# a-to-the-5/Simple-MapReduce-Search-Engine-Information-Retrieval-

Measured on AMD Instinct MI355X. Metric: index build GB/s of text (top-10 queries/sec in 'query'), higher is better.
Workload: dtype u8 text / int32 postings / f64 weights

## Files before the change

### simple-mapreduce-search-engine-information-retrieval-_amd/csrc/sme_api.hip

```cpp
#include <hip/hip_runtime.h>
#include <string.h>

#include <sstream>
#include <string>
#include <vector>

#include <algorithm>
#include <system_error>
#include <thread>

#include "sme_feedback.hpp"
#include "sme_internal.hpp"

namespace {
thread_local std::string g_err;

int fail(int code, const std::string &msg) {
  g_err = msg;
  return code;
}

template <typename F>
int guard(F &&f) {
  try {
// ... 245 lines not shown
      range(0, 2);
      cx->opt_query_kernel = v;
    } else if (n == "heavy_div") {
      range(0, int64_t(1) << 40);
      cx->opt_heavy_div = v;
    } else if (n == "seed_tiles") {
      range(0, 8);
      cx->opt_seed_tiles = v;
    } else if (n == "query_order") {
      range(0, 1);
      cx->opt_query_order = v;
    } else if (n == "agg_two_pass") {
      range(0, 1);
      cx->opt_agg_two_pass = v;
    } else if (n == "agg_grid") {
      range(0, int64_t(1) << 30);
      cx->opt_agg_grid = v;
    } else if (n == "tok_grid") {
      range(1, int64_t(1) << 30);
      cx->opt_tok_grid = v;
    } else if (n == "cand_cap") {
      range(1, 2048);
      cx->opt_cand_cap = v;
    } else if (n == "win_sample") {
      range(0, 1);
      cx->opt_win_sample = v;
    } else if (n == "win_stage_min") {
      range(0, int64_t(1) << 20);
      cx->opt_win_stage_min = v;
    } else if (n == "kgram_rank") {
      range(0, 1);
      cx->opt_kgram_rank = v;
    } else if (n == "win_slice") {
      range(0, int64_t(1) << 30);
      cx->opt_win_slice = v;
    } else if (n == "seed_m") {
      range(0, 4096);
      cx->opt_seed_m = v;
    } else if (n == "query_table_budget") {
      range(0, int64_t(1) << 50);
      cx->opt_query_budget = v;
    } else if (n == "corpus_keep_bytes") {
      range(0, int64_t(1) << 50);
      cx->opt_corpus_keep = v;
    } else if (n == "raw_load_pct") {
      range(10, 90);
      cx->opt_raw_load_pct = v;
    } else if (n == "docid_terms") {
      range(0, 1);
      cx->opt_docid_terms = v;
    } else if (n == "sort_digit_bits") {
      if (v != 0) range(6, 11);
      cx->opt_sort_bits = v;
    } else if (n == "docid_split") {
      range(0, 2);
      cx->opt_docid_split = v;
    } else if (n == "wild_scan") {
      range(0, 1);
      cx->opt_wild_scan = v;
    } else if (n == "wild_chunk") {
      range(64, 4096);
      if (v % 64) throw sme::Error(SME_EINVAL, "option " + n + " must be a multiple of 64");
      cx->opt_wild_chunk = v;
    } else if (n == "fuzzy_scan") {
      range(0, 1);
      cx->opt_fuzzy_scan = v;
    } else if (n == "bool_chunk") {
      range(64, 4096);
      if (v % 64) throw sme::Error(SME_EINVAL, "option " + n + " must be a multiple of 64");
      cx->opt_bool_chunk = v;
    } else if (n == "bool_driver") {
      range(0, 1);
      cx->opt_bool_driver = v;
    } else if (n == "positions") {
      range(0, 1);
      cx->opt_positions = v;
    } else if (n == "struct_narrow") {
      range(0, 1);
      cx->opt_struct_narrow = v;
    } else if (n == "fb_slots") {
      if (!sme::feedback::legal_slots(v))
        throw sme::Error(SME_EINVAL, "option " + n + " must be a power of two in [" +
                                         std::to_string(sme::feedback::kMinSlots) + ", " +
                                         std::to_string(sme::feedback::kMaxSlots) + "]");
      cx->opt_fb_slots = v;
    } else {
      throw sme::Error(SME_EINVAL, "unknown option " + n);
    }
  });
}

static void ctx_release(sme_ctx *cx) {
  (void)hipSetDevice(cx->device);
  (void)hipDeviceSynchronize();
  if (cx->own_stream) (void)hipStreamDestroy(cx->own_stream);
  if (cx->aux_stream) (void)hipStreamDestroy(cx->aux_stream);
  if (cx->ev_fork) (void)hipEventDestroy(cx->ev_fork);
  if (cx->ev_join) (void)hipEventDestroy(cx->ev_join);
  for (hipEvent_t e : cx->prof_events) (void)hipEventDestroy(e);
  for (auto &b : cx->h_stage)
    if (b) (void)hipHostFree(b);
  delete cx;
}

void sme_destroy(sme_ctx *cx) {
  if (!cx) return;
// ... 952 lines not shown
```

### simple-mapreduce-search-engine-information-retrieval-_amd/csrc/sme_build.hip

```cpp
#include <hip/hip_runtime.h>
#include <limits.h>
#include <math.h>
#include <stdio.h>
#include <stdlib.h>
#include <string.h>

#include <algorithm>
#include <memory>
#include <chrono>

#include "sme_internal.hpp"
#include "sme_text.hpp"
#include "sme_trec.hpp"

namespace sme {


template <typename B>
__device__ bool doc_tag_valid(const B &t, int64_t p, const char *tag, int tl) {
  int chain = 0;
  int64_t x = p;
  for (;;) {
    int64_t q = -1;
    for (int j = 1; j < tl; j++) {
// ... 1952 lines not shown
    raw_nout[s] = 1;
  }
}

__global__ void k_code_to_merged(int32_t *raw_term, uint64_t rcap, int32_t *multi, int64_t nmulti,
                                 const int64_t *wrank, const int64_t *drank) {
  const uint64_t gs = (uint64_t)gridDim.x * blockDim.x;
  for (uint64_t s = blockIdx.x * (uint64_t)blockDim.x + threadIdx.x; s < rcap + (uint64_t)nmulti; s += gs) {
    int32_t *p = s < rcap ? raw_term + s : multi + (s - rcap);
    const int32_t v = *p;
    if (v >= 0) *p = (int32_t)((v & kDocCode) ? drank[v & ~kDocCode] : wrank[v]);
  }
}
__global__ void k_dsplit_flags(const int32_t *dk_rec, int64_t nR, uint8_t *flag) {
  for (int64_t i = blockIdx.x * (int64_t)blockDim.x + threadIdx.x; i < nR; i += (int64_t)gridDim.x * blockDim.x)
    flag[i] = dk_rec[i] >= 0;
}
__global__ void k_dsplit_gather(const int32_t *idx, const unsigned long long *nd, const int32_t *dk_rec,
                                const uint32_t *dv_rec, uint32_t *dk, uint32_t *dv, unsigned long long *desc) {
  const int64_t n = (int64_t)*nd;
  for (int64_t q = blockIdx.x * (int64_t)blockDim.x + threadIdx.x; q < n; q += (int64_t)gridDim.x * blockDim.x) {
    dk[q] = (uint32_t)dk_rec[idx[q]];
    dv[q] = dv_rec[idx[q]];
    if (q > 0 && dk_rec[idx[q - 1]] > dk_rec[idx[q]]) atomicAdd(desc, 1ull);
  }
}
__global__ void k_word_shift(const int64_t *wrank, int64_t Vw, const uint32_t *dk, int64_t Nd, uint2 *ws) {
  for (int64_t i = blockIdx.x * (int64_t)blockDim.x + threadIdx.x; i < Vw; i += (int64_t)gridDim.x * blockDim.x) {
    const uint32_t below = (uint32_t)(wrank[i] - i);
    int64_t lo = 0, hi = Nd;
    while (lo < hi) {
      const int64_t m = (lo + hi) >> 1;
      if (dk[m] < below) lo = m + 1;
      else hi = m;
    }
    ws[i] = make_uint2((uint32_t)lo, (uint32_t)wrank[i]);
  }
}
__device__ __forceinline__ int64_t words_below(int64_t j, const int64_t *drank, const int64_t *wrank, int64_t Vw,
                                               const uint2 *ws, const int64_t *off, int64_t Pw) {
  const int64_t x = drank[j] - j;
  return x < Vw ? off[wrank[x]] - (int64_t)ws[x].x : Pw;
}
__global__ void k_docid_place(const uint32_t *dk, const uint32_t *dv, int64_t Nd, const int64_t *drank,
                              const int64_t *wrank, int64_t Vw, const uint2 *ws, const int64_t *off, int64_t Pw,
                              int64_t dmin, uint32_t F, int32_t *docno, int32_t *tf, uint32_t *key, const double *lut,
                              double idf, double *w) {
  for (int64_t q = blockIdx.x * (int64_t)blockDim.x + threadIdx.x; q < Nd; q += (int64_t)gridDim.x * blockDim.x) {
    const int64_t j = dk[q];
    const int64_t p = q + words_below(j, drank, wrank, Vw, ws, off, Pw);
    const uint32_t v = dv[q];
    docno[p] = (int32_t)((int64_t)(v / F) + dmin);
    tf[p] = (int32_t)(v % F);
    key[p] = (uint32_t)drank[j];
    if (w) w[p] = __dmul_rn(lut[v % F], idf);
  }
}
__global__ void k_docid_off(const uint32_t *dk, int64_t Nd, int64_t Vd, const int64_t *drank, const int64_t *wrank,
                            int64_t Vw, const uint2 *ws, int64_t Pw, int64_t *off) {
  for (int64_t j = blockIdx.x * (int64_t)blockDim.x + threadIdx.x; j < Vd; j += (int64_t)gridDim.x * blockDim.x) {
    int64_t lo = 0, hi = Nd;
    while (lo < hi) {
      const int64_t m = (lo + hi) >> 1;
      if ((int64_t)dk[m] < j) lo = m + 1;
      else hi = m;
    }
    off[drank[j]] = lo + words_below(j, drank, wrank, Vw, ws, off, Pw);
  }
}

constexpr int kAggNT = 256;
constexpr int kAggCap = 4096;
constexpr int kAggLimit = 3072;

__device__ __forceinline__ uint32_t hash32(uint32_t x) {
  x ^= x >> 16;
  x *= 0x7feb352dU;
  x ^= x >> 15;
  x *= 0x846ca68bU;
  x ^= x >> 16;
  return x;
}

__device__ __forceinline__ bool agg_insert(int32_t *keys, int32_t *cnt, uint32_t cap_mask, int32_t term,
                                           int32_t *distinct, int32_t limit) {
  uint32_t h = hash32((uint32_t)term) & cap_mask;
  for (uint32_t probe = 0; probe <= cap_mask; probe++) {
    int32_t old = atomicCAS(&keys[h], -1, term);
    if (old == -1) {
      int32_t d = atomicAdd(distinct, 1);
      atomicAdd(&cnt[h], 1);
      return d < limit;
    }
    if (old == term) {
      atomicAdd(&cnt[h], 1);
      return true;
    }
    h = (h + 1) & cap_mask;
  }
  return false;
}

struct AggIn {
  const uint64_t *rs;
  const uint32_t *tokstream;
  const int32_t *ntok;
  const int32_t *raw_term;
// ... 1685 lines not shown
  int64_t Pm = P;
  int32_t max_tf = 1;
  bool packed = false;
  int64_t dmin = 0;
  uint32_t F = 0;
  if (ai.v32 != nullptr || ai.rec_val != nullptr) {
    max_tf = std::max<int32_t>(1, h_mtf);
    packed = true;
    dmin = ai.dmin;
    F = ai.F;
  } else if (P > 0 && !dup_docno && K == 1) {
    SME_HIP(hipMemsetAsync(mtf, 0, sizeof(unsigned int), st));
    const int h_init[2] = {INT_MAX, INT_MIN};
    SME_HIP(hipMemcpyAsync(dmn, h_init, sizeof h_init, hipMemcpyHostToDevice, st));
    hipLaunchKernelGGL(k_pair_stats, dim3(grid_for(P, 256, 2048)), dim3(256), 0, st, p_val, P, mtf);
    hipLaunchKernelGGL(k_docno_range, dim3(grid_for(nR, 256, 1024)), dim3(256), 0, st, docno, nR, dmn, dmx);
    unsigned int h_m = d2h(mtf, st);
    int h_r[2];
    SME_HIP(hipMemcpyAsync(h_r, dmn, sizeof h_r, hipMemcpyDeviceToHost, st));
    SME_HIP(hipStreamSynchronize(st));
    const uint64_t Fq = (uint64_t)h_m + 1, D = (uint64_t)((int64_t)h_r[1] - (int64_t)h_r[0] + 1);
    max_tf = std::max<int32_t>(1, (int32_t)h_m);
    packed = D * Fq < (1ull << 32) && tbits + bits_for((uint64_t)max_tf) <= 32;
    dmin = h_r[0];
    F = (uint32_t)Fq;
  }
  int32_t *docno_d = nullptr, *tf_d = nullptr;
  int64_t *off = nullptr;
  std::vector<double> early_lut;
  bool weights_fused = false;
  if (packed) {
    const int sort_bits = cx->opt_sort_bits > 0 ? (int)cx->opt_sort_bits : (Pw > (int64_t(1) << 30) ? 8 : 11);
    uint32_t *v32 = ai.v32;
    if (ai.rec_val != nullptr) {
      if (term_sort_passes(tbits, sort_bits) >= 3) v32 = W[W_PVAL].as<uint32_t>(P + 1);
    } else if (v32 == nullptr) {
      v32 = reinterpret_cast<uint32_t *>(W[W_T1].as<uint64_t>(P + 1));
      hipLaunchKernelGGL(k_pack_pairs, dim3(grid_for(P)), dim3(256), 0, st, p_val, P, dmin, F, v32);
    }
    uint32_t *v32s = W[W_T2].as<uint32_t>(P + 1);
    docno_d = ix->d_docno_d.as<int32_t>(P + 1);
    tf_d = ix->d_tf_d.as<int32_t>(P + 1);
    uint32_t *rscr = W[W_RADIX].as<uint32_t>(term_sort_scratch(P) / sizeof(uint32_t) + 1);
    double *wf = nullptr;
    if (ix->idf_mode == SME_IDF_REFERENCE && P > 0) {
      early_lut.assign((size_t)max_tf + 1, 0.0);
      for (int i = 1; i <= max_tf; i++) early_lut[(size_t)i] = 1.0 + log((double)i);
      SME_HIP(hipMemcpyAsync(ix->d_lut.as<double>(max_tf + 1), early_lut.data(), early_lut.size() * sizeof(double),
                             hipMemcpyHostToDevice, st));
      wf = ix->d_w.as<double>(P + 1);
      weights_fused = true;
    }
    const double idf_r = log10((double)(std::max<int64_t>(nR, 0) / 1));
    key_s = term_sort(p_term, v32, key_s, v32s, sort_nrec, sort_reg, sort_xoff, Pw, tbits, dmin, F, docno_d, tf_d, rscr,
                      st, wf ? (const double *)ix->d_lut.p : nullptr, idf_r, wf, sort_bits, xw, P, ai.rec_val,
                      ai.tf_shift);
    off = ix->d_off.as<int64_t>(Vi + 1);
    SME_HIP(hipMemsetAsync(off, 0, (Vi + 1) * sizeof(int64_t), st));
    if (!split) {
      hipLaunchKernelGGL(k_term_offsets<false>, dim3(grid_for(P)), dim3(256), 0, st, key_s, P, off, Vi);
    } else {
      hipLaunchKernelGGL(k_term_offsets<true>, dim3(grid_for(P)), dim3(256), 0, st, key_s, P, off, Vi);
      hipLaunchKernelGGL(k_docid_off, dim3(grid_for(Vd)), dim3(256), 0, st, dk, Nd, Vd, (const int64_t *)drank,
                         (const int64_t *)wrank_all, Vw, xw, Pw, off);
      if (Nd > 0)
        hipLaunchKernelGGL(k_docid_place, dim3(grid_for(Nd)), dim3(256), 0, st, dk, dv, Nd, (const int64_t *)drank,
                           (const int64_t *)wrank_all, Vw, xw, off, Pw, dmin, F, docno_d, tf_d, key_s,
                           wf ? (const double *)ix->d_lut.p : nullptr, idf_r, wf);
    }
    SME_CHECK_LAUNCH();
  } else {
    uint64_t *val_s = W[W_T1].as<uint64_t>(P + 1);
    if (P > 0)
      sort_pairs_v64<uint32_t>(p_term, key_s, p_val, val_s, P, tbits, cx->ws[120], cx->ws[121], cx->ws[122], st);
    if (dup_docno && P > 0) {
      uint64_t *ck = W[W_PVAL].as<uint64_t>(P), *ck2 = W[W_T2].as<uint64_t>(P);
      int32_t *tfv = reinterpret_cast<int32_t *>(W[W_PTERM].as<uint32_t>(P)), *tf2 = W[W_T3].as<int32_t>(P);
      hipLaunchKernelGGL(k_dup_keys, dim3(grid_for(P)), dim3(256), 0, st, key_s, val_s, P, ck, tfv);
      int64_t *nout = reinterpret_cast<int64_t *>(cnt + 10);
      reduce_by_key_sum(ck, tfv, P, ck2, tf2, nout, cx->ws[120], cx->ws[121], cx->ws[23], st);
      Pm = d2h(nout, st);
      hipLaunchKernelGGL(k_dup_unpack, dim3(grid_for(Pm)), dim3(256), 0, st, ck2, tf2, Pm, key_s, val_s);
    }
    off = ix->d_off.as<int64_t>(Vi + 1);
    SME_HIP(hipMemsetAsync(off, 0, (Vi + 1) * sizeof(int64_t), st));
    if (Pm > 0) hipLaunchKernelGGL(k_term_offsets<false>, dim3(grid_for(Pm)), dim3(256), 0, st, key_s, Pm, off, Vi);
    docno_d = ix->d_docno_d.as<int32_t>(Pm + 1);
    tf_d = ix->d_tf_d.as<int32_t>(Pm + 1);
    if (Pm > 0) hipLaunchKernelGGL(k_unpack_vals, dim3(grid_for(Pm)), dim3(256), 0, st, val_s, Pm, docno_d, tf_d);
    SME_CHECK_LAUNCH();
    if (Pm > 0) {
      int32_t *mx = reinterpret_cast<int32_t *>(cnt + 11);
      reduce_max<int32_t>(tf_d, Pm, mx, st);
      max_tf = std::max(1, d2h(mx, st));
    }
  }
  ix->P = Pm;
  const int64_t PP = Pm;
  prof.mark("sort_term");

  ix->max_tf = max_tf;
  {
    std::vector<double> lut(max_tf + 1, 0.0);
    for (int i = 1; i <= max_tf; i++) lut[i] = 1.0 + log((double)i);
    double *d_lut = ix->d_lut.as<double>(max_tf + 1);
    SME_HIP(hipMemcpyAsync(d_lut, lut.data(), lut.size() * sizeof(double), hipMemcpyHostToDevice, st));
    const int64_t Nn = std::max<int64_t>(nR, 0);
    ix->idf_N = Nn;
    double idf_ref = idf_value(Nn, 1);
    int64_t sdf = (int64_t)std::sqrt((double)std::max<int64_t>(Nn, 1)) + 1;
    std::vector<double> by_df(sdf + 1), by_q(Nn / std::max<int64_t>(sdf, 1) + 2);
    for (int64_t d = 1; d <= sdf; d++) by_df[d] = idf_value(Nn, d);
    for (size_t q = 0; q < by_q.size(); q++) by_q[q] = idf_value((int64_t)q, 1);
    double *d_bydf = W[W_U16].as<double>(by_df.size() + by_q.size());
    double *d_byq = d_bydf + by_df.size();
    SME_HIP(hipMemcpyAsync(d_bydf, by_df.data(), by_df.size() * sizeof(double), hipMemcpyHostToDevice, st));
    SME_HIP(hipMemcpyAsync(d_byq, by_q.data(), by_q.size() * sizeof(double), hipMemcpyHostToDevice, st));
    double *idf = ix->d_idf.as<double>(Vi + 1);
    if (Vi > 0)
      hipLaunchKernelGGL(k_term_idf, dim3(grid_for(Vi)), dim3(256), 0, st, off, Vi, idf_ref, Nn, nullptr, d_bydf, sdf,
                         d_byq, ix->idf_mode, idf);
// ... 123 lines not shown
```

### simple-mapreduce-search-engine-information-retrieval-_amd/csrc/sme_internal.hpp

```cpp
#pragma once
#include <hip/hip_runtime.h>
#include <math.h>
#include <stdint.h>

#include <memory>
#include <string>
#include <vector>

#include "sme_common.hpp"
#include "sme_result.hpp"

struct sme_ctx {
  sme::BufPool pool;
  sme_config cfg{};
  int device = 0;
  hipStream_t own_stream = nullptr;
  hipStream_t aux_stream = nullptr;
  hipEvent_t ev_fork = nullptr, ev_join = nullptr;
  std::vector<hipEvent_t> prof_events;
  sme::DevBuf map_chars, map_off;
  int64_t map_n = 0;
  bool has_map = false;
  sme::DevBuf map_slots;
  uint64_t map_mask = 0;
  bool map_hash_ok = false;
  sme::DevBuf ws[128];
  sme::DevBuf cub_tmp;
  sme::DevBuf q_gates;
  uint64_t vocab_long_cap = 0, vocab_ovf_cap = 0, raw_cap_hint = 0, lt_cap_hint = 0;
  std::string profile_json;
  std::vector<std::pair<std::string, float>> last_profile;
  std::vector<uint8_t> mapping_out;
  std::vector<int32_t> h_wlist;
  float last_query_ms = -1.0f;
  float last_query_prep_ms = -1.0f;
  float last_query_index_ms = -1.0f;
  bool last_query_tiled = false;
  const char *last_query_name = "k_query";
  float last_query_seed_ms = 0.0f, last_query_final_ms = 0.0f, last_query_total_ms = 0.0f;
  int64_t last_query_overflow = 0;
  int64_t last_query_fallback = 0;
  int64_t last_query_stages = 0;
  int64_t last_query_slices = 0;
  bool last_query_split = false;
  int64_t opt_query_kernel = 0;
  int64_t opt_heavy_div = 128;
  int64_t opt_seed_tiles = 4;
  int64_t opt_query_order = 1;
  int64_t opt_agg_two_pass = 0;
  int64_t opt_agg_grid = 0;
  int64_t opt_tok_grid = 5120;
  int64_t opt_raw_load_pct = 40;
  int64_t opt_docid_terms = 1;
  int64_t opt_sort_bits = 0;
  int64_t opt_docid_split = 1;
  int64_t opt_cand_cap = 1024;
  int64_t opt_seed_m = 64;
  int64_t opt_kgram_rank = 0;
  int64_t opt_win_slice = 0;
  int64_t opt_win_sample = 1;
  int64_t opt_win_stage_min = 0;
  int64_t opt_query_budget = 0;
  int64_t opt_wild_scan = 0;
  int64_t opt_wild_chunk = 1024;
  int64_t opt_fuzzy_scan = 0;
  int64_t opt_bool_chunk = 1024;
  int64_t opt_bool_driver = 0;
  int64_t opt_positions = 0;
  int64_t opt_struct_narrow = 1;
  int64_t opt_fb_slots = 4096;
  int64_t opt_corpus_keep = int64_t(16) << 30;
  void *h_stage[2] = {nullptr, nullptr};
  size_t h_stage_cap = 0;
  sme::DevBuf h_corpus_dev;
  int live_indexes = 0;
  bool destroyed = false;
};

struct sme_index {
  sme_ctx *ctx = nullptr;
  int K = 1, R = 1, idf_mode = 0;
  int job = 0;
  int64_t cg_ngrams = 0, cg_pairs = 0;
  int64_t N = 0, V = 0, P = 0;
  int64_t Vt = 0;
  int32_t max_tf = 0;
  int64_t dmin = 0, dmax = -1;
  sme::DevBuf d_term_off;
  sme::DevBuf d_term_chars;
  sme::DevBuf d_off;
  sme::DevBuf d_docno_d;
  sme::DevBuf d_tf_d;
  sme::DevBuf d_w;
  sme::DevBuf d_idf;
  sme::DevBuf d_gram;
  sme::DevBuf d_lut;
  sme::DevBuf d_docno_o;
  sme::DevBuf d_tf_o;
  sme::DevBuf d_rec_docno;
  sme::DevBuf d_rec_first;
  bool records_only = false;
  bool from_records = false;
  sme::DevBuf d_ser;
  std::vector<int64_t> part_start;
  bool ser_ready = false;
  float ser_ms = 0.0f;
  std::vector<std::unique_ptr<uint8_t[]>> h_parts;
// ... 64 lines not shown
  std::vector<hipEvent_t> *pool;
  std::vector<std::pair<std::string, hipEvent_t>> ev;
  Prof(hipStream_t s, std::vector<hipEvent_t> *p) : st(s), pool(p) { mark("start"); }
  ~Prof() {
    for (auto &e : ev) pool->push_back(e.second);
  }
  void mark(const char *name) {
    hipEvent_t e;
    if (!pool->empty()) {
      e = pool->back();
      pool->pop_back();
    } else {
      SME_HIP(hipEventCreate(&e));
    }
    ev.emplace_back(name, e);
    last_stage() = name;
    SME_HIP(hipEventRecord(e, st));
  }
  std::vector<std::pair<std::string, float>> finish() {
    SME_HIP(hipEventSynchronize(ev.back().second));
    std::vector<std::pair<std::string, float>> out;
    for (size_t i = 1; i < ev.size(); i++) {
      float ms = 0;
      SME_HIP(hipEventElapsedTime(&ms, ev[i - 1].second, ev[i].second));
      out.emplace_back(ev[i].first, ms);
    }
    float tot = 0;
    SME_HIP(hipEventElapsedTime(&tot, ev.front().second, ev.back().second));
    out.emplace_back("total", tot);
    for (auto &p : ev) pool->push_back(p.second);
    ev.clear();
    return out;
  }
};

struct RecordSpans {
  uint64_t *rs, *re;
  int64_t nR;
  uint64_t *C;
  int64_t nC;
  int lt_attempts;
};
void build_docid_hash(sme_ctx *cx, bool distinct, hipStream_t st);
RecordSpans find_records(sme_ctx *cx, const uint8_t *d_text, uint64_t n, hipStream_t st, Prof *prof);
void split_points(sme_ctx *cx, const uint8_t *d_text, uint64_t n, int world, uint64_t *h_cuts, hipStream_t st);
void number_documents(sme_ctx *cx, const uint8_t *d_text, uint64_t n, hipStream_t st, std::vector<uint8_t> &out);
sme_index *build_index(sme_ctx *cx, const uint8_t *d_text, uint64_t n, hipStream_t st, int job = 0);
void chargram_stage(sme_ctx *cx, sme_index *ix, const int32_t *tstream, int64_t M, int64_t V, const int64_t *term_off,
                    const uint16_t *term_chars, hipStream_t st, Prof *prof);
uint32_t *term_sort(uint32_t *k0, uint32_t *v0, uint32_t *k1, uint32_t *v1, int64_t nrec, const int64_t *reg,
                    const int64_t *xoff, int64_t P, int bits, int64_t dmin, uint32_t F, int32_t *docno, int32_t *tf,
                    uint32_t *counts, hipStream_t st, const double *lut = nullptr, double idf = 0.0,
                    double *w = nullptr, int maxbits = 11, const uint2 *xw = nullptr, int64_t Pout = 0,
                    const uint32_t *rec_val = nullptr, int tf_shift = 0);
int term_sort_passes(int bits, int maxbits);
size_t term_sort_scratch(int64_t P);
template <typename K>
uint32_t *kv_sort(K *k0, uint32_t *v0, K *k1, uint32_t *v1, int64_t n, int bits, uint32_t *scratch, hipStream_t st,
                  bool keys_out = false);
size_t kv_sort_scratch(int64_t n);
template <typename T>
void excl_scan(const T *in, T *out, int64_t n, DevBuf &scratch, hipStream_t st);
void select_flagged(const uint8_t *flag, int64_t n, int32_t *out, int32_t *d_count, DevBuf &s1, DevBuf &s2,
                    hipStream_t st);
template <typename K>
void sort_pairs(K *keys_in, K *keys_out, uint32_t *vals_in, uint32_t *vals_out, int64_t n, int bits, DevBuf &radix,
                hipStream_t st);
template <typename K>
void sort_pairs_v64(K *keys_in, K *keys_out, const uint64_t *vals_in, uint64_t *vals_out, int64_t n, int bits,
                    DevBuf &ia, DevBuf &ib, DevBuf &radix, hipStream_t st);
template <typename T>
void reduce_max(const T *in, int64_t n, T *d_max, hipStream_t st);
void reduce_by_key_sum(const uint64_t *keys, const int32_t *vals, int64_t n, uint64_t *ukeys, int32_t *sums,
                       int64_t *d_runs, DevBuf &flags, DevBuf &pos, DevBuf &scan, hipStream_t st);
constexpr int kTfSortMaxTf = 1023;
void tf_sort_segments(const int64_t *off, int64_t V, int64_t P, const int32_t *docno_d, const int32_t *tf_d,
                      int max_tf, int32_t *docno_o, int32_t *tf_o, DevBuf &lists, DevBuf &tiles, DevBuf &tcnt, DevBuf &scan,
                      unsigned long long *nseg, hipStream_t st, hipStream_t aux_stream, hipEvent_t ev_fork,
                      hipEvent_t ev_join);
void serialize_index(sme_index *ix, hipStream_t st);
void pack_pieces(sme_index *ix, int world, uint8_t *d_out, uint64_t *sizes, hipStream_t st);
sme_index *merge_pieces(sme_ctx *cx, const uint8_t *d_blobs, const uint64_t *sizes, int np, hipStream_t st);
void reweight_index(sme_index *ix, int64_t N, const int64_t *d_gdf, hipStream_t st,
                    const uint32_t *d_term_of = nullptr);
sme_index *load_records(sme_ctx *cx, const uint8_t *d_records, const uint64_t *part_offsets, int np, hipStream_t st);
void prepare_queries(sme_index *ix, hipStream_t st);
void query_topk(sme_index *ix, const int32_t *d_terms, const int64_t *d_qoff, int nq, int k,
                int32_t *d_out_docno, double *d_out_score, uint32_t *d_out_tie, hipStream_t st, int tie_bits = 0);
void query_topk_java7(sme_index *ix, const int32_t *d_terms, const int64_t *d_qoff, int nq, int k,
                      int32_t *d_out_docno, double *d_out_score, uint32_t *d_out_tie, hipStream_t st);
void tokenize_string(sme_ctx *cx, const uint8_t *h_utf8, size_t n, std::vector<std::vector<uint16_t>> &out,
                     hipStream_t st);
void term_fingerprints(sme_index *ix, uint64_t *d_out, hipStream_t st);
void dfx_pack(sme_ctx *cx, const uint64_t *fp, const int64_t *df, int64_t n, int world, uint64_t *sfp, int64_t *sdf,
              int64_t *pos, int64_t *h_counts, hipStream_t st);
void dfx_sum(sme_ctx *cx, const uint64_t *fp, const int64_t *df, int64_t n, int64_t *out, int64_t *h_distinct,
             hipStream_t st);
void dfx_unpack(const int64_t *ret, const int64_t *pos, int64_t n, int64_t *out, hipStream_t st);
void merge_rows(const double *s, const int32_t *d, const uint32_t *t, int64_t rows, int m, int k, int32_t *od,
                double *os, uint32_t *ot, hipStream_t st);
int64_t count_shared_keys(sme_ctx *cx, const uint64_t *rows, int64_t n, hipStream_t st);
void lookup_terms(sme_index *ix, const std::vector<std::vector<uint16_t>> &terms, int32_t *ids,
                  hipStream_t st);
void prepare_wildcards(sme_index *ix, hipStream_t st);
void expand_wildcards(sme_index *ix, const uint8_t *patterns, const int64_t *offs, int n, hipStream_t st);
void suggest_terms(sme_index *ix, const uint8_t *words, const int64_t *offs, int n, int max_dist, int m,
                   hipStream_t st);
// ... 26 lines not shown
```

### simple-mapreduce-search-engine-information-retrieval-_amd/csrc/sme_sort.hip

```cpp
#include <hip/hip_runtime.h>

#include "sme_internal.hpp"

namespace sme {
namespace {

#ifndef SME_RSNT
#define SME_RSNT 512
#endif
constexpr int kRsNT = SME_RSNT;
constexpr int kRsWaves = kRsNT / 64;
constexpr int kRsIPL = 16;
constexpr int kRsTile = kRsNT * kRsIPL;
constexpr int kRsWaveItems = 64 * kRsIPL;
constexpr int kRsMaxBits = 11;
constexpr int kRsMaxBins = 1 << kRsMaxBits;
constexpr int kRsBPT = kRsMaxBins / kRsNT;
constexpr int kRsGroups = 1024;
constexpr int kRsScanSums = 1024;

struct RsGroups {
  int64_t tpg;
  int G;
};
static RsGroups rs_groups(int64_t ntiles) {
  const int64_t tpg = std::max<int64_t>(4, (ntiles + kRsGroups - 1) / kRsGroups);
  const int64_t g = (ntiles + tpg - 1) / tpg;
  return RsGroups{tpg, (int)((g + 15) / 16 * 16)};
}

struct Gather {
  const int64_t *reg, *xoff, *crec;
  int64_t nrec;
  const uint32_t *rval;
  int tf_shift;
};
__device__ __forceinline__ void gather_start(const Gather &g, int64_t x, int64_t &rec, int64_t &nx, int64_t &dl) {
  rec = g.crec[x >> 10];
  nx = g.xoff[rec + 1];
  dl = g.reg[rec] - g.xoff[rec];
}
__device__ __forceinline__ int64_t gather_pos(const Gather &g, int64_t x, int64_t &rec, int64_t &nx, int64_t &dl) {
  while (x >= nx) {
    rec++;
    nx = g.xoff[rec + 1];
    dl = g.reg[rec] - g.xoff[rec];
  }
  return x + dl;
}
constexpr int kGRec = 48;
__device__ __forceinline__ int64_t gather_table(const Gather &g, int64_t x0, int lane, int64_t *gx, int64_t *gdl,
                                                uint32_t *gv = nullptr) {
  const int64_t rec0 = g.crec[x0 >> 10];
  const int64_t r = rec0 + lane;
  if (lane < kGRec) {
    gx[lane] = r <= g.nrec ? g.xoff[r] : INT64_MAX;
    gdl[lane] = r < g.nrec ? g.reg[r] - g.xoff[r] : 0;
    if (gv) gv[lane] = r < g.nrec ? g.rval[r] : 0u;
  }
  if (lane == 0) gx[kGRec] = rec0 + kGRec <= g.nrec ? g.xoff[rec0 + kGRec] : INT64_MAX;
  __builtin_amdgcn_fence(__ATOMIC_SEQ_CST, "wavefront");
  __builtin_amdgcn_wave_barrier();
  return rec0;
}
__device__ __forceinline__ int64_t gather_at(const Gather &g, int64_t x, int &j, const int64_t *gx, const int64_t *gdl,
                                             int64_t rec0, uint32_t *jr = nullptr) {
  while (j < kGRec - 1 && x >= gx[j + 1]) j++;
  if (x < gx[j + 1]) {
    if (jr) *jr = (uint32_t)j;
    return x + gdl[j];
  }
  int64_t rec = rec0 + kGRec - 1, nx = g.xoff[rec + 1], dl = g.reg[rec] - g.xoff[rec];
  const int64_t p = gather_pos(g, x, rec, nx, dl);
  if (jr) *jr = (uint32_t)(rec - rec0);
  return p;
}
__global__ void k_rs_chunk_rec(const int64_t *__restrict__ xoff, int64_t nrec, int64_t P, int64_t *__restrict__ crec) {
  for (int64_t c = blockIdx.x * (int64_t)blockDim.x + threadIdx.x; (c << 10) < P; c += (int64_t)gridDim.x * blockDim.x) {
    const int64_t x = c << 10;
    int64_t lo = 0, hi = nrec;
    while (hi - lo > 1) {
      const int64_t m = (lo + hi) >> 1;
      if (xoff[m] <= x) lo = m;
      else hi = m;
    }
    crec[c] = lo;
  }
}

__global__ __launch_bounds__(kRsNT) void k_rs_count(const uint32_t *__restrict__ key, int64_t P, int shift,
                                                    int nbins, uint32_t *__restrict__ counts, Gather g) {
  __shared__ uint32_t h[kRsMaxBins];
  const int tid = threadIdx.x;
  for (int b = tid; b < nbins; b += kRsNT) h[b] = 0;
  __syncthreads();
  const int64_t t0 = (int64_t)blockIdx.x * kRsTile;
  const uint32_t mask = (uint32_t)nbins - 1u;
  const int64_t n = min((int64_t)kRsTile, P - t0);
  if (g.reg != nullptr) {
    __shared__ int64_t gx_all[kRsWaves][kGRec + 1], gdl_all[kRsWaves][kGRec];
    const int lane = tid & 63, w = tid >> 6;
    const int64_t wb = t0 + (int64_t)w * kRsWaveItems;
    if (wb < P) {
      const int64_t rec0 = gather_table(g, wb, lane, gx_all[w], gdl_all[w]);
      int j = 0;
      uint32_t kk[kRsIPL];
#pragma unroll
      for (int s = 0; s < kRsIPL; s++) {
        const int64_t x = wb + s * 64 + lane;
        kk[s] = x < P ? key[gather_at(g, x, j, gx_all[w], gdl_all[w], rec0)] : 0u;
      }
#pragma unroll
      for (int s = 0; s < kRsIPL; s++)
        if (wb + s * 64 + lane < P) atomicAdd(&h[(kk[s] >> shift) & mask], 1u);
    }
  } else if (n == kRsTile) {
    const uint4 *k4 = reinterpret_cast<const uint4 *>(key + t0);
#pragma unroll
    for (int i = 0; i < kRsIPL / 4; i++) {
// ... 39 lines not shown
    for (int c = 0; c < 4; c++) s += x[c].x + x[c].y + x[c].z + x[c].w;
    uint32_t incl = s;
    for (int o = 1; o < 64; o <<= 1) {
      const uint32_t u = __shfl_up(incl, o, 64);
      if (lane >= o) incl += u;
    }
    if (lane == 63) ws[w] = incl;
    uint4 xn[4];
    load(r0 + 16 * kRsNT, xn);
    __syncthreads();
    uint32_t wb = carry, tot = 0;
    for (int j = 0; j < kRsWaves; j++) {
      const uint32_t t = ws[j];
      if (j < w) wb += t;
      tot += t;
    }
    uint32_t run = wb + incl - s;
    if (i0 < n) {
#pragma unroll
      for (int c = 0; c < 4; c++) {
        uint4 y;
        y.x = run;
        run += x[c].x;
        y.y = run;
        run += x[c].y;
        y.z = run;
        run += x[c].z;
        y.w = run;
        run += x[c].w;
        reinterpret_cast<uint4 *>(a + i0)[c] = y;
      }
    }
    carry += tot;
    __syncthreads();
#pragma unroll
    for (int c = 0; c < 4; c++) x[c] = xn[c];
  }
}

__global__ __launch_bounds__(kRsNT) void k_rs_colscan(uint32_t *__restrict__ counts, int64_t ntiles, int nbins,
                                                      int64_t tpg, int G, const uint32_t *__restrict__ gsum) {
  const int g = blockIdx.x;
  const int64_t ta = (int64_t)g * tpg, tb = min(ntiles, ta + tpg);
  for (int b = threadIdx.x; b < nbins; b += kRsNT) {
    uint32_t run = gsum[(int64_t)b * G + g];
    for (int64_t t = ta; t < tb; t++) {
      const uint32_t c = counts[t * nbins + b];
      counts[t * nbins + b] = run;
      run += c;
    }
  }
}

template <bool LAST, bool PACK>
__global__ __launch_bounds__(kRsNT) void k_rs_scatter(const uint32_t *__restrict__ key, const uint32_t *__restrict__ val,
                                                      int64_t P, int shift, int nbits,
                                                      const uint32_t *__restrict__ offs, uint32_t *__restrict__ okey,
                                                      uint32_t *__restrict__ oval, int32_t *__restrict__ odocno,
                                                      int32_t *__restrict__ otf, int64_t dmin, uint32_t F,
                                                      Gather g, const double *__restrict__ lut, double idf,
                                                      double *__restrict__ ow, const uint2 *__restrict__ xw) {
  __shared__ uint16_t wc[kRsWaves * kRsMaxBins];
  __shared__ uint32_t gd[kRsMaxBins];
  __shared__ uint32_t stage[kRsTile];
  __shared__ uint32_t ws[kRsWaves];
  const int tid = threadIdx.x, lane = tid & 63, w = tid >> 6;
  const int nbins = 1 << nbits;
  const uint32_t mask = (uint32_t)nbins - 1u;
  const int64_t per = (int64_t)(gridDim.x >> 3);
  const int64_t tile = (int64_t)(blockIdx.x & 7) * per + (blockIdx.x >> 3);
  const int64_t t0 = tile * kRsTile;
  if (t0 >= P) return;
  const int n = (int)min((int64_t)kRsTile, P - t0);
  for (int i = tid; i < kRsWaves * kRsMaxBins / 2; i += kRsNT) reinterpret_cast<uint32_t *>(wc)[i] = 0u;
  __syncthreads();
  uint16_t *mine = wc + w * kRsMaxBins;
  const int wb = w * kRsWaveItems;
  const uint64_t lt = (1ull << lane) - 1ull;
  uint32_t k[kRsIPL], v[kRsIPL], pos[kRsIPL];
  if (g.reg != nullptr) {
    __shared__ int64_t gx_all[kRsWaves][kGRec + 1], gdl_all[kRsWaves][kGRec];
    __shared__ uint32_t gv_all[kRsWaves][kGRec];
    uint32_t *gv = PACK ? gv_all[w] : nullptr;
    int64_t rec0 = 0;
    if (wb < n) rec0 = gather_table(g, t0 + wb, lane, gx_all[w], gdl_all[w], gv);
    int j = 0;
    if (PACK) {
      const uint32_t kmask = g.tf_shift >= 32 ? 0xFFFFFFFFu : (1u << g.tf_shift) - 1u;
#pragma unroll
      for (int s = 0; s < kRsIPL; s++) {
        const int i = wb + s * 64 + lane;
        k[s] = 0u;
        v[s] = 0u;
        if (i < n) k[s] = key[gather_at(g, t0 + i, j, gx_all[w], gdl_all[w], rec0, &v[s])];
      }
#pragma unroll
      for (int s = 0; s < kRsIPL; s++) {
        const uint32_t wd = k[s], jr = v[s];
        k[s] = wd & kmask;
        if (wb + s * 64 + lane < n)
          v[s] = (jr < (uint32_t)kGRec ? gv[jr] : g.rval[rec0 + jr]) + (uint32_t)((uint64_t)wd >> g.tf_shift);
      }
    } else {
#pragma unroll
      for (int s = 0; s < kRsIPL; s++) {
        const int i = wb + s * 64 + lane;
        k[s] = 0u;
// ... 38 lines not shown
    uint32_t tc[kRsBPT];
    uint32_t s2 = 0;
#pragma unroll
    for (int q = 0; q < kRsBPT; q++) {
      tc[q] = 0;
      if (b0 + q < nbins) {
#pragma unroll
        for (int x = 0; x < kRsWaves; x++) tc[q] += wc[x * kRsMaxBins + b0 + q];
      }
      s2 += tc[q];
    }
    uint32_t incl = s2;
    for (int o = 1; o < 64; o <<= 1) {
      const uint32_t u = __shfl_up(incl, o, 64);
      if (lane >= o) incl += u;
    }
    if (lane == 63) ws[w] = incl;
    __syncthreads();
    uint32_t ex = incl - s2;
    for (int j = 0; j < w; j++) ex += ws[j];
#pragma unroll
    for (int q = 0; q < kRsBPT; q++) {
      if (b0 + q < nbins) {
        uint32_t r = ex;
        gd[b0 + q] = offs[tile * nbins + b0 + q] - r;
#pragma unroll
        for (int x = 0; x < kRsWaves; x++) {
          const uint32_t c = wc[x * kRsMaxBins + b0 + q];
          wc[x * kRsMaxBins + b0 + q] = (uint16_t)r;
          r += c;
        }
      }
      ex += tc[q];
    }
  }
  __syncthreads();
#pragma unroll
  for (int s = 0; s < kRsIPL; s++) {
    if (wb + s * 64 + lane >= n) continue;
    pos[s] += mine[(k[s] >> shift) & mask];
    stage[pos[s]] = k[s];
  }
  __syncthreads();
  uint32_t dst[kRsIPL];
#pragma unroll
  for (int j = 0; j < kRsIPL; j++) {
    const int p = j * kRsNT + tid;
    if (p < n) {
      const uint32_t kk = stage[p];
      dst[j] = gd[(kk >> shift) & mask] + (uint32_t)p;
      if (LAST && xw) {
        const uint2 x = xw[kk];
        dst[j] += x.x;
        okey[dst[j]] = x.y;
      } else {
        okey[dst[j]] = kk;
      }
    }
  }
  __syncthreads();
#pragma unroll
  for (int s = 0; s < kRsIPL; s++)
    if (wb + s * 64 + lane < n) stage[pos[s]] = v[s];
  __syncthreads();
#pragma unroll
  for (int j = 0; j < kRsIPL; j++) {
    const int p = j * kRsNT + tid;
    if (p < n) {
      const uint32_t vv = stage[p];
      if (LAST) {
        odocno[dst[j]] = (int32_t)((int64_t)(vv / F) + dmin);
        otf[dst[j]] = (int32_t)(vv % F);
        if (ow) ow[dst[j]] = __dmul_rn(lut[vv % F], idf);
      } else {
        oval[dst[j]] = vv;
      }
    }
  }
}

template <typename K>
__global__ __launch_bounds__(kRsNT) void k_kv_count(const K *__restrict__ key, int64_t n, int shift, int nbins,
                                                    uint32_t *__restrict__ counts) {
  __shared__ uint32_t h[kRsMaxBins];
  const int tid = threadIdx.x;
  for (int b = tid; b < nbins; b += kRsNT) h[b] = 0;
  __syncthreads();
  const int64_t t0 = (int64_t)blockIdx.x * kRsTile;
  const int m = (int)min((int64_t)kRsTile, n - t0);
  const uint32_t mask = (uint32_t)nbins - 1u;
  for (int i = tid; i < m; i += kRsNT) atomicAdd(&h[(uint32_t)(key[t0 + i] >> shift) & mask], 1u);
  __syncthreads();
  for (int b = tid; b < nbins; b += kRsNT) counts[(int64_t)blockIdx.x * nbins + b] = h[b];
}

template <typename K, bool KEYS>
__global__ __launch_bounds__(kRsNT) void k_kv_scatter(const K *__restrict__ key, const uint32_t *__restrict__ val,
                                                      int64_t n_all, int shift, int nbits,
                                                      const uint32_t *__restrict__ offs, K *__restrict__ okey,
                                                      uint32_t *__restrict__ oval) {
  __shared__ uint16_t wc[kRsWaves * kRsMaxBins];
  __shared__ uint32_t gd[kRsMaxBins];
  __shared__ uint32_t stage[kRsTile];
  __shared__ uint32_t ws[kRsWaves];
  const int tid = threadIdx.x, lane = tid & 63, w = tid >> 6;
  const int nbins = 1 << nbits;
  const uint32_t mask = (uint32_t)nbins - 1u;
  const int64_t per = (int64_t)(gridDim.x >> 3);
  const int64_t tile = (int64_t)(blockIdx.x & 7) * per + (blockIdx.x >> 3);
  const int64_t t0 = tile * kRsTile;
  if (t0 >= n_all) return;
  const int n = (int)min((int64_t)kRsTile, n_all - t0);
  for (int i = tid; i < kRsWaves * kRsMaxBins / 2; i += kRsNT) reinterpret_cast<uint32_t *>(wc)[i] = 0u;
  __syncthreads();
  uint16_t *mine = wc + w * kRsMaxBins;
  const int wb = w * kRsWaveItems;
  const uint64_t lt = (1ull << lane) - 1ull;
  K k[kRsIPL];
  uint32_t v[kRsIPL], pos[kRsIPL];
#pragma unroll
  for (int s = 0; s < kRsIPL; s++) {
    const int i = wb + s * 64 + lane;
    const bool ok = i < n;
    k[s] = ok ? key[t0 + i] : (K)0;
    v[s] = ok ? val[t0 + i] : 0u;
  }
#pragma unroll
  for (int s = 0; s < kRsIPL; s++) {
    const bool ok = wb + s * 64 + lane < n;
    const uint32_t d = (uint32_t)(k[s] >> shift) & mask;
// ... 153 lines not shown
    const int64_t i = t0 + j * kScNT + threadIdx.x;
    st[P(j * kScNT + threadIdx.x)] = i < n ? in[i] : (T)0;
  }
  __syncthreads();
  T x[kScIPT], s = 0;
#pragma unroll
  for (int j = 0; j < kScIPT; j++) {
    x[j] = st[P(threadIdx.x * kScIPT + j)];
    s += x[j];
  }
  T tot;
  T run = carry[blockIdx.x] + sc_block_excl<T>(s, ws, &tot);
#pragma unroll
  for (int j = 0; j < kScIPT; j++) {
    st[P(threadIdx.x * kScIPT + j)] = run;
    run += x[j];
  }
  __syncthreads();
#pragma unroll
  for (int j = 0; j < kScIPT; j++) {
    const int64_t i = t0 + j * kScNT + threadIdx.x;
    if (i < n) out[i] = st[P(j * kScNT + threadIdx.x)];
  }
}

__global__ void k_flags_i64(const uint8_t *__restrict__ f, int64_t n, int64_t *__restrict__ v) {
  for (int64_t i = blockIdx.x * (int64_t)blockDim.x + threadIdx.x; i < n; i += (int64_t)gridDim.x * blockDim.x)
    v[i] = f[i] ? 1 : 0;
}
__global__ void k_select_scatter(const uint8_t *__restrict__ f, const int64_t *__restrict__ pos, int64_t n,
                                 int32_t *__restrict__ out, int32_t *__restrict__ count) {
  for (int64_t i = blockIdx.x * (int64_t)blockDim.x + threadIdx.x; i < n; i += (int64_t)gridDim.x * blockDim.x) {
    if (f[i]) out[pos[i]] = (int32_t)i;
    if (i == n - 1) *count = (int32_t)(pos[i] + (f[i] ? 1 : 0));
  }
}

void rs_scan(uint32_t *gsum, int64_t n, uint32_t *sums, hipStream_t st) {
  if (n <= 16 * 4 * kRsNT) {
    hipLaunchKernelGGL(k_rs_scan, dim3(1), dim3(kRsNT), 0, st, gsum, (int)n);
    return;
  }
  const int64_t nt = (n + kScTile - 1) / kScTile;
  hipLaunchKernelGGL(k_sc_sums<uint32_t>, dim3((unsigned)nt), dim3(kScNT), 0, st, gsum, n, sums);
  hipLaunchKernelGGL(k_sc_carry<uint32_t>, dim3(1), dim3(kScNT), 0, st, sums, nt);
  hipLaunchKernelGGL(k_sc_apply<uint32_t>, dim3((unsigned)nt), dim3(kScNT), 0, st, gsum, gsum, n, sums);
}

}

uint32_t *term_sort(uint32_t *k0, uint32_t *v0, uint32_t *k1, uint32_t *v1, int64_t nrec, const int64_t *reg,
                    const int64_t *xoff, int64_t P, int bits, int64_t dmin, uint32_t F, int32_t *docno, int32_t *tf,
                    uint32_t *counts, hipStream_t st, const double *lut, double idf, double *w, int maxbits,
                    const uint2 *xw, int64_t Pout, const uint32_t *rec_val, int tf_shift) {
  if (P <= 0) return k0;
  if (P > 0xFFFFFFFFll) throw Error(SME_ELIMIT, "term sort of more than 2^32 pairs");
  bits = std::max(bits, 1);
  maxbits = std::min(std::max(maxbits, 1), kRsMaxBits);
  const int npass = term_sort_passes(bits, maxbits);
  const int64_t ntiles = (P + kRsTile - 1) / kRsTile;
  const RsGroups rg = rs_groups(ntiles);
  const int64_t tpg = rg.tpg;
  const int G = rg.G;
  uint32_t *gsum = counts + ntiles * kRsMaxBins;
  Gather g0{nullptr, nullptr, nullptr, 0, nullptr, 0};
  if (reg != nullptr) {
    int64_t *crec = reinterpret_cast<int64_t *>(gsum + kRsMaxBins * kRsGroups + kRsScanSums);
    const int64_t nch = (P + 1023) >> 10;
    hipLaunchKernelGGL(k_rs_chunk_rec, dim3((unsigned)std::min<int64_t>((nch + 255) / 256, 4096)), dim3(256), 0, st,
                       xoff, nrec, P, crec);
    g0 = Gather{reg, xoff, crec, nrec, rec_val, tf_shift};
  }
  int shift = 0;
  for (int p = 0; p < npass; p++) {
    const Gather g = p == 0 ? g0 : Gather{nullptr, nullptr, nullptr, 0, nullptr, 0};
#ifdef SME_RS_LOFIRST
    const int nb = (bits - shift) / (npass - p);
#else
    const int nb = (bits - shift + (npass - p) - 1) / (npass - p);
#endif
    const int nbins = 1 << nb;
    const bool last = p == npass - 1;
    hipLaunchKernelGGL(k_rs_count, dim3((unsigned)ntiles), dim3(kRsNT), 0, st, k0, P, shift, nbins, counts, g);
    hipLaunchKernelGGL(k_rs_colsum, dim3(G), dim3(kRsNT), 0, st, counts, ntiles, nbins, tpg, G, gsum);
    rs_scan(gsum, (int64_t)nbins * G, gsum + kRsMaxBins * kRsGroups, st);
    hipLaunchKernelGGL(k_rs_colscan, dim3(G), dim3(kRsNT), 0, st, counts, ntiles, nbins, tpg, G, gsum);
    const unsigned sgrid = (unsigned)(8 * ((ntiles + 7) / 8));
    if (last && xw)
      SME_HIP(hipMemsetAsync(k1, 0xFF, (size_t)Pout * sizeof(uint32_t), st));
    const bool pack = g.reg != nullptr && g.rval != nullptr;
    auto *scatter = last ? (pack ? k_rs_scatter<true, true> : k_rs_scatter<true, false>)
                         : (pack ? k_rs_scatter<false, true> : k_rs_scatter<false, false>);
    if (last)
      hipLaunchKernelGGL(scatter, dim3(sgrid), dim3(kRsNT), 0, st, k0, v0, P, shift, nb, counts, k1, nullptr, docno, tf,
                         dmin, F, g, lut, idf, w, xw);
    else
      hipLaunchKernelGGL(scatter, dim3(sgrid), dim3(kRsNT), 0, st, k0, v0, P, shift, nb, counts, k1, v1, nullptr,
                         nullptr, dmin, F, g, nullptr, 0.0, nullptr, nullptr);
    SME_CHECK_LAUNCH();
    std::swap(k0, k1);
    std::swap(v0, v1);
    shift += nb;
  }
  return k0;
}

int term_sort_passes(int bits, int maxbits) {
  const int mb = std::min(std::max(maxbits, 1), kRsMaxBits);
  return (std::max(bits, 1) + mb - 1) / mb;
}

size_t term_sort_scratch(int64_t P) {
  const int64_t ntiles = (std::max<int64_t>(P, 1) + kRsTile - 1) / kRsTile;
  return (size_t)(ntiles * kRsMaxBins + (int64_t)kRsMaxBins * kRsGroups + kRsScanSums) * sizeof(uint32_t) +
         (size_t)(((std::max<int64_t>(P, 1) + 1023) >> 10) + 1) * sizeof(int64_t);
}
template <typename K>
uint32_t *kv_sort(K *k0, uint32_t *v0, K *k1, uint32_t *v1, int64_t n, int bits, uint32_t *scratch, hipStream_t st,
                  bool keys_out) {
  if (n <= 1) return v0;
  if (n > 0xFFFFFFFFll) throw Error(SME_ELIMIT, "sort of more than 2^32 pairs");
  bits = std::min(std::max(bits, 1), (int)(8 * sizeof(K)));
  const int npass = (bits + kRsMaxBits - 1) / kRsMaxBits;
  const int64_t ntiles = (n + kRsTile - 1) / kRsTile;
  const RsGroups rg = rs_groups(ntiles);
  const int64_t tpg = rg.tpg;
  const int G = rg.G;
  uint32_t *counts = scratch, *gsum = scratch + ntiles * kRsMaxBins;
  int shift = 0;
  for (int p = 0; p < npass; p++) {
    const int nb = (bits - shift + (npass - p) - 1) / (npass - p);
    const int nbins = 1 << nb;
    hipLaunchKernelGGL(k_kv_count<K>, dim3((unsigned)ntiles), dim3(kRsNT), 0, st, k0, n, shift, nbins, counts);
    hipLaunchKernelGGL(k_rs_colsum, dim3(G), dim3(kRsNT), 0, st, counts, ntiles, nbins, tpg, G, gsum);
    rs_scan(gsum, (int64_t)nbins * G, gsum + kRsMaxBins * kRsGroups, st);
    hipLaunchKernelGGL(k_rs_colscan, dim3(G), dim3(kRsNT), 0, st, counts, ntiles, nbins, tpg, G, gsum);
    const unsigned sgrid = (unsigned)(8 * ((ntiles + 7) / 8));
    if (p == npass - 1 && !keys_out)
      hipLaunchKernelGGL((k_kv_scatter<K, false>), dim3(sgrid), dim3(kRsNT), 0, st, k0, v0, n, shift, nb, counts,
                         k1, v1);
    else
      hipLaunchKernelGGL((k_kv_scatter<K, true>), dim3(sgrid), dim3(kRsNT), 0, st, k0, v0, n, shift, nb, counts, k1,
                         v1);
    SME_CHECK_LAUNCH();
    std::swap(k0, k1);
    std::swap(v0, v1);
    shift += nb;
  }
  return v0;
}
template uint32_t *kv_sort<uint64_t>(uint64_t *, uint32_t *, uint64_t *, uint32_t *, int64_t, int, uint32_t *,
// ... 134 lines not shown
```

Measured before the change: 177.4.

## Derive term offsets from radix-sort last-pass tables instead of scanning sorted keys

Adds a kernel that computes per-term posting offsets directly from the final radix-sort pass's per-tile prefix counts. It only processes tiles where the lower-digit prefix changes, so the separate k_term_offsets pass over all sorted keys is no longer needed. When weights are fused and tf is small, the final scatter also skips writing sorted keys and the key memset, which saves memory traffic. In exchange the code is more complex and leans on subtle invariants about the sort's digit layout, and later stages that read keys may break if they still depend on them.

```diff
diff --git a/simple-mapreduce-search-engine-information-retrieval-_amd/csrc/sme_api.hip b/simple-mapreduce-search-engine-information-retrieval-_amd/csrc/sme_api.hip
--- a/simple-mapreduce-search-engine-information-retrieval-_amd/csrc/sme_api.hip
+++ b/simple-mapreduce-search-engine-information-retrieval-_amd/csrc/sme_api.hip
@@ -321,6 +321,9 @@
     } else if (n == "sort_digit_bits") {
       if (v != 0) range(6, 11);
       cx->opt_sort_bits = v;
+    } else if (n == "term_off_tables") {
+      range(0, 1);
+      cx->opt_term_off_tables = v;
     } else if (n == "docid_split") {
       range(0, 2);
       cx->opt_docid_split = v;
diff --git a/simple-mapreduce-search-engine-information-retrieval-_amd/csrc/sme_build.hip b/simple-mapreduce-search-engine-information-retrieval-_amd/csrc/sme_build.hip
--- a/simple-mapreduce-search-engine-information-retrieval-_amd/csrc/sme_build.hip
+++ b/simple-mapreduce-search-engine-information-retrieval-_amd/csrc/sme_build.hip
@@ -2028,7 +2028,7 @@
     const uint32_t v = dv[q];
     docno[p] = (int32_t)((int64_t)(v / F) + dmin);
     tf[p] = (int32_t)(v % F);
-    key[p] = (uint32_t)drank[j];
+    if (key) key[p] = (uint32_t)drank[j];
     if (w) w[p] = __dmul_rn(lut[v % F], idf);
   }
 }
@@ -3820,21 +3820,25 @@
       weights_fused = true;
     }
     const double idf_r = log10((double)(std::max<int64_t>(nR, 0) / 1));
+    const bool off_tables = cx->opt_term_off_tables != 0;
+    const bool want_keys = !(off_tables && weights_fused && max_tf <= kTfSortMaxTf);
+    off = ix->d_off.as<int64_t>(Vi + 1);
+    SME_HIP(hipMemsetAsync(off, 0, (Vi + 1) * sizeof(int64_t), st));
     key_s = term_sort(p_term, v32, key_s, v32s, sort_nrec, sort_reg, sort_xoff, Pw, tbits, dmin, F, docno_d, tf_d, rscr,
                       st, wf ? (const double *)ix->d_lut.p : nullptr, idf_r, wf, sort_bits, xw, P, ai.rec_val,
-                      ai.tf_shift);
-    off = ix->d_off.as<int64_t>(Vi + 1);
-    SME_HIP(hipMemsetAsync(off, 0, (Vi + 1) * sizeof(int64_t), st));
+                      ai.tf_shift, off_tables ? off : nullptr, split ? Vw : Vi, Vi, want_keys);
     if (!split) {
-      hipLaunchKernelGGL(k_term_offsets<false>, dim3(grid_for(P)), dim3(256), 0, st, key_s, P, off, Vi);
+      if (!off_tables)
+        hipLaunchKernelGGL(k_term_offsets<false>, dim3(grid_for(P)), dim3(256), 0, st, key_s, P, off, Vi);
     } else {
-      hipLaunchKernelGGL(k_term_offsets<true>, dim3(grid_for(P)), dim3(256), 0, st, key_s, P, off, Vi);
+      if (!off_tables)
+        hipLaunchKernelGGL(k_term_offsets<true>, dim3(grid_for(P)), dim3(256), 0, st, key_s, P, off, Vi);
       hipLaunchKernelGGL(k_docid_off, dim3(grid_for(Vd)), dim3(256), 0, st, dk, Nd, Vd, (const int64_t *)drank,
                          (const int64_t *)wrank_all, Vw, xw, Pw, off);
       if (Nd > 0)
         hipLaunchKernelGGL(k_docid_place, dim3(grid_for(Nd)), dim3(256), 0, st, dk, dv, Nd, (const int64_t *)drank,
-                           (const int64_t *)wrank_all, Vw, xw, off, Pw, dmin, F, docno_d, tf_d, key_s,
-                           wf ? (const double *)ix->d_lut.p : nullptr, idf_r, wf);
+                           (const int64_t *)wrank_all, Vw, xw, off, Pw, dmin, F, docno_d, tf_d,
+                           want_keys ? key_s : nullptr, wf ? (const double *)ix->d_lut.p : nullptr, idf_r, wf);
     }
     SME_CHECK_LAUNCH();
   } else {
diff --git a/simple-mapreduce-search-engine-information-retrieval-_amd/csrc/sme_internal.hpp b/simple-mapreduce-search-engine-information-retrieval-_amd/csrc/sme_internal.hpp
--- a/simple-mapreduce-search-engine-information-retrieval-_amd/csrc/sme_internal.hpp
+++ b/simple-mapreduce-search-engine-information-retrieval-_amd/csrc/sme_internal.hpp
@@ -53,6 +53,7 @@
   int64_t opt_raw_load_pct = 40;
   int64_t opt_docid_terms = 1;
   int64_t opt_sort_bits = 0;
+  int64_t opt_term_off_tables = 1;
   int64_t opt_docid_split = 1;
   int64_t opt_cand_cap = 1024;
   int64_t opt_seed_m = 64;
@@ -223,7 +224,8 @@
                     const int64_t *xoff, int64_t P, int bits, int64_t dmin, uint32_t F, int32_t *docno, int32_t *tf,
                     uint32_t *counts, hipStream_t st, const double *lut = nullptr, double idf = 0.0,
                     double *w = nullptr, int maxbits = 11, const uint2 *xw = nullptr, int64_t Pout = 0,
-                    const uint32_t *rec_val = nullptr, int tf_shift = 0);
+                    const uint32_t *rec_val = nullptr, int tf_shift = 0, int64_t *off_out = nullptr, int64_t V = 0,
+                    int64_t vend = 0, bool write_keys = true);
 int term_sort_passes(int bits, int maxbits);
 size_t term_sort_scratch(int64_t P);
 template <typename K>
diff --git a/simple-mapreduce-search-engine-information-retrieval-_amd/csrc/sme_sort.hip b/simple-mapreduce-search-engine-information-retrieval-_amd/csrc/sme_sort.hip
--- a/simple-mapreduce-search-engine-information-retrieval-_amd/csrc/sme_sort.hip
+++ b/simple-mapreduce-search-engine-information-retrieval-_amd/csrc/sme_sort.hip
@@ -18,6 +18,7 @@
 constexpr int kRsBPT = kRsMaxBins / kRsNT;
 constexpr int kRsGroups = 1024;
 constexpr int kRsScanSums = 1024;
+constexpr int kRsOffTiles = 16;
 
 struct RsGroups {
   int64_t tpg;
@@ -65,6 +66,10 @@
 }
 __device__ __forceinline__ int64_t gather_at(const Gather &g, int64_t x, int &j, const int64_t *gx, const int64_t *gdl,
                                              int64_t rec0, uint32_t *jr = nullptr) {
+#ifdef SME_RS_GATHER_CEIL
+  if (jr) *jr = 0u;
+  return x + gdl[0];
+#endif
   while (j < kGRec - 1 && x >= gx[j + 1]) j++;
   if (x < gx[j + 1]) {
     if (jr) *jr = (uint32_t)j;
@@ -210,7 +215,7 @@
   }
 }
 
-template <bool LAST, bool PACK>
+template <bool LAST, bool PACK, bool KEYS = true>
 __global__ __launch_bounds__(kRsNT) void k_rs_scatter(const uint32_t *__restrict__ key, const uint32_t *__restrict__ val,
                                                       int64_t P, int shift, int nbits,
                                                       const uint32_t *__restrict__ offs, uint32_t *__restrict__ okey,
@@ -355,8 +360,8 @@
       if (LAST && xw) {
         const uint2 x = xw[kk];
         dst[j] += x.x;
-        okey[dst[j]] = x.y;
-      } else {
+        if (KEYS) okey[dst[j]] = x.y;
+      } else if (KEYS) {
         okey[dst[j]] = kk;
       }
     }
@@ -379,6 +384,105 @@
         oval[dst[j]] = vv;
       }
     }
+  }
+}
+
+__global__ __launch_bounds__(kRsNT) void k_rs_term_off(const uint32_t *__restrict__ key, int64_t P, int shift, int nbits,
+                                                       const uint32_t *__restrict__ offs, int64_t V,
+                                                       const uint2 *__restrict__ xw, int64_t *__restrict__ off,
+                                                       int64_t vend, int64_t pend) {
+  __shared__ uint32_t ks[kRsTile];
+  __shared__ uint16_t sp[kRsTile];
+  __shared__ uint32_t hist[kRsMaxBins];
+  __shared__ uint32_t rc[kRsIPL * kRsWaves + 1];
+  __shared__ uint32_t act;
+  const int tid = threadIdx.x, lane = tid & 63, w = tid >> 6;
+  const int nbins = 1 << nbits;
+  const uint32_t mask = (uint32_t)nbins - 1u;
+  const uint32_t lmask = (1u << shift) - 1u;
+  if (blockIdx.x == 0 && tid == 0) off[vend] = pend;
+  if (P <= 0) return;
+  int64_t tile = 0;
+  auto emit = [&](uint32_t L) {
+    for (int d = tid; d < nbins; d += kRsNT) {
+      const uint64_t k = ((uint64_t)d << shift) | L;
+      if (k < (uint64_t)V) {
+        const int64_t o = (int64_t)offs[tile * nbins + d] + hist[d];
+        if (xw) {
+          const uint2 x = xw[k];
+          off[x.y] = o + x.x;
+        } else {
+          off[k] = o;
+        }
+      }
+    }
+  };
+  if (shift == 0) {
+    for (int b = tid; b < nbins; b += kRsNT) hist[b] = 0;
+    __syncthreads();
+    emit(0u);
+    return;
+  }
+  if (tid == 0) act = 0u;
+  __syncthreads();
+  if (tid < kRsOffTiles) {
+    const int64_t a0 = ((int64_t)blockIdx.x * kRsOffTiles + tid) * kRsTile;
+    if (a0 < P) {
+      const int64_t last = min(a0 + kRsTile, P) - 1;
+      if (a0 == 0 || (key[a0 - 1] & lmask) != (key[last] & lmask)) atomicOr(&act, 1u << tid);
+    }
+  }
+  __syncthreads();
+  const uint64_t lt = (1ull << lane) - 1ull;
+  for (uint32_t todo = act; todo != 0u; todo &= todo - 1u) {
+    tile = (int64_t)blockIdx.x * kRsOffTiles + (__ffs(todo) - 1);
+    const int64_t t0 = tile * kRsTile;
+    const int n = (int)min((int64_t)kRsTile, P - t0);
+    const uint32_t lprev = t0 > 0 ? key[t0 - 1] & lmask : 0u;
+    for (int b = tid; b < nbins; b += kRsNT) hist[b] = 0;
+    for (int p = tid; p < n; p += kRsNT) ks[p] = key[t0 + p];
+    __syncthreads();
+    uint32_t mine = 0;
+#pragma unroll
+    for (int j = 0; j < kRsIPL; j++) {
+      const int p = j * kRsNT + tid;
+      bool f = false;
+      if (p < n) f = (ks[p] & lmask) != (p > 0 ? ks[p - 1] & lmask : lprev) || (p == 0 && t0 == 0);
+      const uint64_t b = (uint64_t)__ballot(f);
+      if (f) mine |= 1u << j;
+      if (lane == 0) rc[j * kRsWaves + w] = (uint32_t)__popcll(b);
+    }
+    __syncthreads();
+    if (w == 0) {
+      const uint32_t a = rc[2 * lane], b = rc[2 * lane + 1];
+      uint32_t incl = a + b;
+      for (int o = 1; o < 64; o <<= 1) {
+        const uint32_t u = __shfl_up(incl, o, 64);
+        if (lane >= o) incl += u;
+      }
+      rc[2 * lane] = incl - a - b;
+      rc[2 * lane + 1] = incl - b;
+      if (lane == 63) rc[kRsIPL * kRsWaves] = incl;
+    }
+    __syncthreads();
+#pragma unroll
+    for (int j = 0; j < kRsIPL; j++) {
+      const bool f = (mine >> j) & 1u;
+      const uint64_t b = (uint64_t)__ballot(f);
+      if (f) sp[rc[j * kRsWaves + w] + (uint32_t)__popcll(b & lt)] = (uint16_t)(j * kRsNT + tid);
+    }
+    __syncthreads();
+    const int ns = (int)rc[kRsIPL * kRsWaves];
+    int pos = 0;
+    for (int si = 0; si < ns; si++) {
+      const int s = sp[si];
+      for (int p = pos + tid; p < s; p += kRsNT) atomicAdd(&hist[(ks[p] >> shift) & mask], 1u);
+      __syncthreads();
+      emit(ks[s] & lmask);
+      __syncthreads();
+      pos = s;
+    }
+    __syncthreads();
   }
 }
 
@@ -638,8 +742,18 @@
 uint32_t *term_sort(uint32_t *k0, uint32_t *v0, uint32_t *k1, uint32_t *v1, int64_t nrec, const int64_t *reg,
                     const int64_t *xoff, int64_t P, int bits, int64_t dmin, uint32_t F, int32_t *docno, int32_t *tf,
                     uint32_t *counts, hipStream_t st, const double *lut, double idf, double *w, int maxbits,
-                    const uint2 *xw, int64_t Pout, const uint32_t *rec_val, int tf_shift) {
-  if (P <= 0) return k0;
+                    const uint2 *xw, int64_t Pout, const uint32_t *rec_val, int tf_shift, int64_t *off_out, int64_t V,
+                    int64_t vend, bool write_keys) {
+  if (vend <= 0) vend = V;
+  const int64_t pend = xw ? Pout : std::max<int64_t>(P, 0);
+  if (P <= 0) {
+    if (off_out) {
+      hipLaunchKernelGGL(k_rs_term_off, dim3(1), dim3(kRsNT), 0, st, nullptr, 0, 0, 1, nullptr, V, xw, off_out, vend,
+                         pend);
+      SME_CHECK_LAUNCH();
+    }
+    return k0;
+  }
   if (P > 0xFFFFFFFFll) throw Error(SME_ELIMIT, "term sort of more than 2^32 pairs");
   bits = std::max(bits, 1);
   maxbits = std::min(std::max(maxbits, 1), kRsMaxBits);
@@ -672,17 +786,21 @@
     rs_scan(gsum, (int64_t)nbins * G, gsum + kRsMaxBins * kRsGroups, st);
     hipLaunchKernelGGL(k_rs_colscan, dim3(G), dim3(kRsNT), 0, st, counts, ntiles, nbins, tpg, G, gsum);
     const unsigned sgrid = (unsigned)(8 * ((ntiles + 7) / 8));
-    if (last && xw)
+    if (last && xw && write_keys)
       SME_HIP(hipMemsetAsync(k1, 0xFF, (size_t)Pout * sizeof(uint32_t), st));
     const bool pack = g.reg != nullptr && g.rval != nullptr;
-    auto *scatter = last ? (pack ? k_rs_scatter<true, true> : k_rs_scatter<true, false>)
-                         : (pack ? k_rs_scatter<false, true> : k_rs_scatter<false, false>);
+    auto *scatter = !last        ? (pack ? k_rs_scatter<false, true> : k_rs_scatter<false, false>)
+                    : write_keys ? (pack ? k_rs_scatter<true, true> : k_rs_scatter<true, false>)
+                                 : (pack ? k_rs_scatter<true, true, false> : k_rs_scatter<true, false, false>);
     if (last)
       hipLaunchKernelGGL(scatter, dim3(sgrid), dim3(kRsNT), 0, st, k0, v0, P, shift, nb, counts, k1, nullptr, docno, tf,
                          dmin, F, g, lut, idf, w, xw);
     else
       hipLaunchKernelGGL(scatter, dim3(sgrid), dim3(kRsNT), 0, st, k0, v0, P, shift, nb, counts, k1, v1, nullptr,
                          nullptr, dmin, F, g, nullptr, 0.0, nullptr, nullptr);
+    if (last && off_out)
+      hipLaunchKernelGGL(k_rs_term_off, dim3(shift == 0 ? 1u : (unsigned)((ntiles + kRsOffTiles - 1) / kRsOffTiles)),
+                         dim3(kRsNT), 0, st, k0, P, shift, nb, counts, V, xw, off_out, vend, pend);
     SME_CHECK_LAUNCH();
     std::swap(k0, k1);
     std::swap(v0, v1);
```

New measurement: 180.6, median of 6. 1.02x the previous value.
